# tud-amr/semantic_dsp_map

Measured on AMD Instinct MI355X. Metric: Mvoxels updated/sec (256^3 grid, 2M particles, VKITTI2 camera; whole hot-path frame), higher is better.
Workload: dtype f32

## Files before the change

include/sdm.h:

```cpp
#ifndef SDM_H_
#define SDM_H_

#include <stddef.h>
#include <stdint.h>

#ifdef __cplusplus
extern "C" {
#endif

typedef struct sdm_map sdm_map;

typedef enum {
  SDM_OK = 0,
  SDM_ERR_INVALID_ARGUMENT = 1,
  SDM_ERR_NO_DEVICE = 2,
  SDM_ERR_HIP = 3,
  SDM_ERR_CAPACITY = 4,
  SDM_ERR_NOT_CONVERGED = 5,
  SDM_ERR_COMM = 6
} sdm_status;

typedef struct {
  int32_t x_n, y_n, z_n;
  int32_t p_n;
// ... 309 lines not shown
                          const float *w, const uint16_t *ts, const uint16_t *track,
                          const uint8_t *label, const uint8_t *status, const uint8_t *forget,
                          const uint16_t *owner);
sdm_status sdm_get_ck_kappa(sdm_map *m, float *out);
sdm_status sdm_get_bin_counts(sdm_map *m, uint32_t *out);
sdm_status sdm_get_bins(sdm_map *m, uint32_t *out, int64_t cap, int64_t *n_out);
sdm_status sdm_get_extrinsic(sdm_map *m, float *out16);

sdm_status sdm_time_occupancy_sweep(sdm_map *m, int32_t iters, float *avg_ms);
sdm_status sdm_debug_fill_dense(sdm_map *m);
sdm_status sdm_debug_fill_dense_ex(sdm_map *m, int32_t mode);
sdm_status sdm_debug_hinted_groups(sdm_map *m, int64_t *n_out);
sdm_status sdm_debug_sweep_lists(sdm_map *m, int32_t mode);
sdm_status sdm_debug_sweep_mode(sdm_map *m, int32_t *mode_out);
sdm_status sdm_debug_alias_cap(sdm_map *m, int32_t cap);

sdm_status sdm_test_scan(const uint32_t *in, uint32_t *out, int64_t n);
sdm_status sdm_test_sort_pairs(const uint32_t *keys_in, const uint32_t *vals_in, uint32_t *keys_out,
                               uint32_t *vals_out, int64_t n, int32_t nbits);

const char *sdm_last_error(void);
const char *sdm_version(void);

#ifdef __cplusplus
}
#endif
#endif
```

semantic_dsp_map_amd/binding.py:

```python
import ctypes as C
import os

import numpy as np

_HERE = os.path.dirname(os.path.abspath(__file__))
LIB_PATH = os.environ.get("SDM_LIB_PATH") or os.path.join(_HERE, "csrc", "libsdm_hip.so")

LABELED_POINT = np.dtype([("x", "<f4"), ("y", "<f4"), ("z", "<f4"), ("sigma", "<f4"),
                          ("track_id", "<u2"), ("label_id", "u1"), ("is_valid", "u1")])
OBJECT_MOVE = np.dtype([("track_id", "<i4"), ("T", "<f4", (16,))])
VOXEL_RESULT = np.dtype([("wsum", "<f4"), ("track", "<u2"), ("label", "u1"), ("occ", "i1")])
POINT = np.dtype([("x", "<f4"), ("y", "<f4"), ("z", "<f4"), ("track", "<u2"), ("label", "u1"), ("occ", "i1")])
POINT_XYZRGB = np.dtype([("x", "<f4"), ("y", "<f4"), ("z", "<f4"), ("one", "<f4"), ("b", "u1"), ("g", "u1"), ("r", "u1"), ("a", "u1"),
                         ("pad", "<u4", (3,))])
assert LABELED_POINT.itemsize == 20 and OBJECT_MOVE.itemsize == 68 and VOXEL_RESULT.itemsize == 8 and POINT.itemsize == 16
SEGMENT_HIT = np.dtype([("t", "<f4"), ("voxel", "<u4"), ("cells", "<i4"), ("track", "<u2"), ("label", "u1"), ("occ", "i1")])
BOX_RESULT = np.dtype([("n_occupied", "<i4"), ("n_free", "<i4"), ("n_unknown", "<i4"), ("first_occupied", "<u4"), ("clipped", "<i4")])
assert SEGMENT_HIT.itemsize == 16 and BOX_RESULT.itemsize == 20
QUERY_ON_DEVICE = 0x1
QUERY_UNKNOWN_BLOCKS = 0x2
DISTANCE_RESULT = np.dtype([("distance", "<f4"), ("gradient", "<f4", (3,)), ("nearest", "<f4", (3,)), ("d2", "<u4"), ("track", "<u2"),
                            ("label", "u1"), ("occ", "i1")])
assert DISTANCE_RESULT.itemsize == 36
ESDF_UNKNOWN_IS_OBSTACLE = 0x1
# ... 161 lines not shown
        "sdm_load_state": [vp] + [vp] * 10,
        "sdm_get_ck_kappa": [vp, vp],
        "sdm_get_bin_counts": [vp, vp],
        "sdm_get_bins": [vp, vp, i64, C.POINTER(i64)],
        "sdm_get_extrinsic": [vp, vp],
        "sdm_time_occupancy_sweep": [vp, i32, C.POINTER(C.c_float)],
        "sdm_set_issue_mode": [vp, i32],
        "sdm_bind_host_thread": [i32],
        "sdm_host_numa_node_early": [i32],
        "sdm_debug_fill_dense": [vp],
        "sdm_debug_fill_dense_ex": [vp, i32],
        "sdm_debug_hinted_groups": [vp, C.POINTER(C.c_int64)],
        "sdm_debug_sweep_lists": [vp, i32],
        "sdm_debug_sweep_mode": [vp, C.POINTER(i32)],
        "sdm_debug_alias_cap": [vp, i32],
        "sdm_test_scan": [vp, vp, i64],
        "sdm_test_sort_pairs": [vp, vp, vp, vp, i64, i32],
    }
    for name, argtypes in sig.items():
        fn = getattr(L, name)
        fn.argtypes = argtypes
        fn.restype = C.c_int
    L.sdm_last_error.restype = C.c_char_p
    L.sdm_version.restype = C.c_char_p
    global HOST_NUMA_NODE
    HOST_NUMA_NODE = L.sdm_bind_host_thread(int(os.environ.get("LOCAL_RANK", "0")))
    _lib = L
    return L


def _ptr(a):
    if a is None:
# ... 410 lines not shown
    def dump_state(self):
        n = self.v_count * self.S
        st = {k: np.empty(n, dt) for k, dt in STATE_FIELDS}
        _check(self.L, self.L.sdm_dump_state(self.h, *[_ptr(st[k]) for k, _ in STATE_FIELDS]), "sdm_dump_state")
        return st

    def load_state(self, st):
        arrs = [np.ascontiguousarray(st[k], dtype=dt) for k, dt in STATE_FIELDS]
        _check(self.L, self.L.sdm_load_state(self.h, *[_ptr(a) for a in arrs]), "sdm_load_state")

    def ck_kappa(self):
        out = np.empty(self.W * self.H, np.float32)
        _check(self.L, self.L.sdm_get_ck_kappa(self.h, _ptr(out)), "sdm_get_ck_kappa")
        return out.reshape(self.H, self.W)

    def bin_counts(self):
        out = np.empty(self.W * self.H, np.uint32)
        _check(self.L, self.L.sdm_get_bin_counts(self.h, _ptr(out)), "sdm_get_bin_counts")
        return out.reshape(self.H, self.W)

    def bins(self):
        n = C.c_int64()
        _check(self.L, self.L.sdm_get_bins(self.h, None, 0, C.byref(n)), "sdm_get_bins")
        out = np.empty(max(n.value, 1), np.uint32)
        _check(self.L, self.L.sdm_get_bins(self.h, _ptr(out), n.value, C.byref(n)), "sdm_get_bins")
        return out[:n.value]

    def extrinsic(self):
        out = np.empty(16, np.float32)
        _check(self.L, self.L.sdm_get_extrinsic(self.h, _ptr(out)), "sdm_get_extrinsic")
# ... 37 lines not shown
def test_scan(a):
    L = load_library()
    a = np.ascontiguousarray(a, dtype=np.uint32)
    out = np.empty_like(a)
    _check(L, L.sdm_test_scan(_ptr(a), _ptr(out), a.size), "sdm_test_scan")
    return out


def test_sort_pairs(keys, vals, nbits):
    L = load_library()
    keys = np.ascontiguousarray(keys, dtype=np.uint32)
    vals = np.ascontiguousarray(vals, dtype=np.uint32)
    ko, vo = np.empty_like(keys), np.empty_like(vals)
    _check(L, L.sdm_test_sort_pairs(_ptr(keys), _ptr(vals), _ptr(ko), _ptr(vo), keys.size, nbits), "sdm_test_sort_pairs")
    return ko, vo
```

semantic_dsp_map_amd/csrc/debug.hip:

```cpp
#include "sdm_map.h"

namespace {

__global__ void k_spin(unsigned long long ticks, unsigned long long *out) {
  const unsigned long long t0 = wall_clock64();
  out[0] = t0;
  while (wall_clock64() - t0 < ticks) __builtin_amdgcn_s_sleep(8);
  out[1] = wall_clock64();
}
__global__ void k_stamp(unsigned long long *out) { *out = wall_clock64(); }

}

extern "C" {

sdm_status sdm_debug_overlap(sdm_map *m, int32_t which, double out_us[2]) {
  if (!m || which < 0 || which > 2 || !out_us) return SDM_ERR_INVALID_ARGUMENT;
  HIP_TRY(hipSetDevice(m->device));
  unsigned long long *d = nullptr, h[3] = {0, 0, 0};
  DevTemps tmp;
  HIP_TRY(tmp.alloc(&d, 3));
  if (which == 2) HIP_TRY(lazy_stream(m->device, &m->s_moves));
  hipStream_t side = which == 0 ? m->s_frustum : (which == 1 ? m->s_birth : m->s_moves);
  HIP_TRY(hipStreamSynchronize(m->stream));
// ... 66 lines not shown
  m->st.alias_cap = (uint32_t)cap;
  return SDM_OK;
}
sdm_status sdm_debug_hinted_groups(sdm_map *m, int64_t *n_out) {
  if (!m || !n_out) return SDM_ERR_INVALID_ARGUMENT;
  HIP_TRY(hipSetDevice(m->device));
  std::vector<uint8_t> h(grp_hint_bytes(m->d.v_count));
  HIP_TRY(hipMemcpyAsync(h.data(), m->st.grp_hint, h.size(), hipMemcpyDeviceToHost, m->stream));
  HIP_TRY(hipStreamSynchronize(m->stream));
  int64_t n = 0;
  for (uint8_t b : h) n += b != 0;
  *n_out = n;
  return SDM_OK;
}

#ifdef SDM_AB_TIMERS
extern "C++" {
namespace sdm {
void debug_timers(unsigned long long *out32, int reset);
void debug_timers_moves(unsigned long long *out, int reset);
}
}
sdm_status sdm_debug_timers(sdm_map *m, unsigned long long *out32, int reset) {
  HIP_TRY(hipSetDevice(m->device));
  HIP_TRY(hipDeviceSynchronize());
  sdm::debug_timers(out32, reset);
  sdm::debug_timers_moves(out32 + 6 * 8192 * 4, reset);
  return SDM_OK;
}
#endif
// ... 21 lines not shown
  HIP_TRY(tmp.alloc(&ka, (size_t)n));
  HIP_TRY(tmp.alloc(&va, (size_t)n));
  HIP_TRY(tmp.alloc(&kb, (size_t)n));
  HIP_TRY(tmp.alloc(&vb, (size_t)n));
  HIP_TRY(tmp.alloc(&scr, sort_scratch_elems((size_t)n) + 16));
  HIP_TRY(hipMemset(scr, 0, (sort_scratch_elems((size_t)n) + 16) * 4));
  HIP_TRY(hipMemcpy(ka, keys_in, (size_t)n * 4, hipMemcpyHostToDevice));
  HIP_TRY(hipMemcpy(va, vals_in, (size_t)n * 4, hipMemcpyHostToDevice));
  int which = radix_sort_pairs(ka, va, kb, vb, (size_t)n, nbits, scr, nullptr);
  HIP_TRY(hipDeviceSynchronize());
  HIP_TRY(hipMemcpy(keys_out, which ? kb : ka, (size_t)n * 4, hipMemcpyDeviceToHost));
  HIP_TRY(hipMemcpy(vals_out, which ? vb : va, (size_t)n * 4, hipMemcpyDeviceToHost));
  return SDM_OK;
}

}
```

semantic_dsp_map_amd/csrc/kernels.hip:

```cpp
#include <algorithm>

#include <type_traits>

#include <hip/hip_ext.h>
#include "sdm_internal.h"
#include "sdm_scratch.h"

#pragma clang fp contract(off)

namespace sdm {

namespace {

constexpr int TPB = 256;

#ifdef SDM_AB_TIMERS
}
__device__ unsigned long long g_dbg[6][8192 * 4];
namespace {
#define DBG_T() wall_clock64()
#define DBG_PUTK(k, i, v) do { if (blockIdx.x < 8192) g_dbg[k][blockIdx.x * 4 + (i)] = (unsigned long long)(v); } while (0)
#define DBG_PUT(i, v) DBG_PUTK(0, i, v)
#define DBG_LANE0(k, i) do { if (threadIdx.x == 0 && threadIdx.y == 0) DBG_PUTK(k, i, DBG_T()); } while (0)
#else
// ... 1701 lines not shown
                                         const sdm_labeled_point &o, float ck) {
  if (finish) {
    const float ckk = ck * flt.p_detect + flt.noise_number;
    sc.ck_kappa[p] = ckk;
    sc.pix4[p] = make_float4(o.x, o.y, o.z, ckk);
    sc.pixt[p] = (uint32_t)o.track_id | (1u << 16);
  } else {
    ck_out[p] = ck;
  }
}

constexpr int BR_TPB = 640;
constexpr int BR_WAVES = BR_TPB / 64;
constexpr int BR_MAXW = 1 << ROW_COL_BITS;
template <int PPT>
__global__ __launch_bounds__(BR_TPB) __attribute__((amdgpu_waves_per_eu(PPT <= 4 ? 5 : 4, PPT <= 4 ? 5 : 4))) void k_bin_rows(Dims d, State st, Scratch sc) {
  static_assert(PPT == 2 || PPT == 4 || PPT * BR_TPB >= BR_MAXW, "eight pixels per thread cover the widest image");
  __shared__ uint32_t pre[BR_MAXW + 1];
  __shared__ uint32_t wave_tot[BR_WAVES];
  __shared__ uint32_t s_base;
  const int r = blockIdx.x;
  DBG_LANE0(2, 0);
  if (r == (int)gridDim.x - 1 && threadIdx.x < 64) alias_compact_wave(st);
  const bool overflow = sc.cnt->overflow != 0;
  const int lane = threadIdx.x & 63, wid = threadIdx.x >> 6;
  const int W = d.W;
  uint32_t c[PPT];
  const int j0 = PPT * (int)threadIdx.x;
#pragma unroll
  for (int u = 0; u < PPT; ++u) c[u] = (!overflow && j0 + u < W) ? sc.bin_count[r * W + j0 + u] : 0u;
  uint32_t sub_n = 0;
  if (threadIdx.x < ROW_SUBS && !overflow) {
    sub_n = sc.row_cnt[(size_t)(r * ROW_SUBS + threadIdx.x) * ROW_CNT_STRIDE];
    if (sub_n > sc.row_cap) sub_n = sc.row_cap;
  }
  uint32_t inc = 0;
#pragma unroll
  for (int u = 0; u < PPT; ++u) inc += c[u];
  const uint32_t mine = inc;
#pragma unroll
  for (int off = 1; off < 64; off <<= 1) {
    const uint32_t t = __shfl_up(inc, off, 64);
    if (lane >= off) inc += t;
  }
  if (lane == 63) wave_tot[wid] = inc;
  __syncthreads();
  uint32_t before = 0, total = 0;
#pragma unroll
  for (int w = 0; w < BR_WAVES; ++w) {
    if (w < wid) before += wave_tot[w];
    total += wave_tot[w];
  }
  {
    uint32_t run = before + inc - mine;
#pragma unroll
    for (int u = 0; u < PPT; ++u) {
      if (j0 + u < W) pre[j0 + u] = run;
      run += c[u];
    }
  }
  if (threadIdx.x == 0) {
    pre[W] = total;
    s_base = total ? atomicAdd(&sc.cnt->n_vis, total) : 0u;
    if (total && (s_base > sc.cap_vis || total > sc.cap_vis - s_base)) {
      sc.cnt->overflow = 1;
      pre[W] = 0;
    }
  }
  uint32_t sub_ex[ROW_SUBS + 1];
  {
    uint32_t run = 0;
#pragma unroll
    for (int k = 0; k < ROW_SUBS; ++k) {
      sub_ex[k] = run;
      run += (uint32_t)__shfl(sub_n, k, 64);
    }
    sub_ex[ROW_SUBS] = run;
  }
  __shared__ uint32_t s_sub[ROW_SUBS + 1];
  if (threadIdx.x == 0) {
#pragma unroll
    for (int k = 0; k <= ROW_SUBS; ++k) s_sub[k] = sub_ex[k];
  }
  __syncthreads();
  const uint32_t base = s_base;
  uint32_t *__restrict__ bs = sc.bin_start + (size_t)r * (W + 1);
  const bool row_over = total != 0 && pre[W] == 0;
  {
    const int h = d.window_half;
#pragma unroll
    for (int u = 0; u < PPT; ++u) {
      const int j = j0 + u;
      if (j < W) {
        const uint32_t n = row_over ? 0u : pre[j + h + 1 > W ? W : j + h + 1] - pre[j - h < 0 ? 0 : j - h];
        sc.row_win[r * W + j] = (uint8_t)(n > 255u ? 255u : n);
      }
    }
  }
  for (int j = threadIdx.x; j <= W; j += BR_TPB) bs[j] = row_over ? 0u : base + pre[j];
  if (total == 0 || row_over) {
    DBG_LANE0(2, 1);
    return;
  }
  const uint32_t n_row = s_sub[ROW_SUBS];
  for (uint32_t g = threadIdx.x; g < n_row; g += BR_TPB) {
    int sub = 0;
#pragma unroll
    for (int k = 1; k < ROW_SUBS; ++k) sub += s_sub[k] <= g ? 1 : 0;
    const uint2 e = sc.row_list[(size_t)(r * ROW_SUBS + sub) * sc.row_cap + (g - s_sub[sub])];
    sc.bin_idx[base + pre[e.y & (uint32_t)(BR_MAXW - 1)] + (e.y >> ROW_COL_BITS)] = e.x;
  }
  __syncthreads();
  const size_t slot_base = (size_t)d.v_begin << d.p_n;
// ... 70 lines not shown
          a[0] = t;
          sift_down(a, 0, end - 1);
        }
      }
    }
    for (uint32_t i = 0; i < n; ++i) {
      const size_t li = (size_t)a[i] - slot_base;
      const float4 q = st.pos4[li];
      const SlotRef sr = slot_ref_li(st, d.p_n, li);
      sc.vp4[s + i] = make_float4(q.x, q.y, q.z, sr.w());
      sc.vtf[s + i] = (uint32_t)sr.track() | ((uint32_t)st.forget[li] << 16);
      sc.vpix[s + i] = p;
    }
  }
  DBG_LANE0(2, 1);
}

__global__ __launch_bounds__(TPB) void k_ck_classify(Dims d, Filter flt, Scratch sc, float *__restrict__ ck_out, int finish) {
  const uint32_t p = blockIdx.x * blockDim.x + threadIdx.x;
  const int W = d.W, H = d.H, h = d.window_half;
  const bool in_image = p < (uint32_t)(W * H);
  const bool overflow = sc.cnt->overflow != 0;
  sdm_labeled_point o;
  o.is_valid = 0;
  uint32_t total = 0;
  if (in_image) {
    o = load_point(sc.fa->cloud, p);
    const int i = (int)p / W;
    uint32_t rw[A7_ROWS];
#pragma unroll
    for (int r = 0; r < A7_ROWS; ++r) {
      const int ni = i + r - h;
      const bool ok = r <= 2 * h && ni >= 0 && ni < H;
      rw[r] = sc.row_win[(int)p + (ok ? (r - h) * W : 0)];
    }
    __builtin_amdgcn_sched_barrier(0);
#pragma unroll
    for (int r = 0; r < A7_ROWS; ++r) {
      const int ni = i + r - h;
      total += (r <= 2 * h && ni >= 0 && ni < H) ? rw[r] : 0u;
    }
  }
  uint8_t cls = CK_DONE;
  if (in_image && o.is_valid && total != 0 && !overflow) cls = total <= CK_LIGHT_MAX ? CK_LIGHT : CK_HEAVY;
  const unsigned long long hm = __ballot(cls == CK_HEAVY);
  if (hm) {
    const uint32_t lane = threadIdx.x & 63u;
    const uint32_t shard = blockIdx.x & (VIS_SHARDS - 1);
    uint32_t base = 0;
    if (lane == 0) base = atomicAdd(&sc.cnt->shard[shard].heavy, (uint32_t)__popcll(hm));
    base = (uint32_t)__shfl((int)base, 0, 64);
    if (cls == CK_HEAVY) sc.ck_heavy[shard * sc.cap_heavy + base + (uint32_t)__popcll(hm & ((1ull << lane) - 1ull))] = p;
  }
  if (!in_image) return;
  if (!finish) {
    sc.pix4[p] = make_float4(o.x, o.y, o.z, 0.f);
    sc.pixt[p] = o.is_valid ? ((uint32_t)o.track_id | (1u << 16)) : 0u;
  }
  if (!o.is_valid) {
    if (finish) sc.pixt[p] = 0;
  } else if (cls == CK_DONE) {
    ck_store(flt, sc, ck_out, finish, (int)p, o, 0.f);
  }
  sc.ck_class[p] = cls;
}


template <bool FAST>
__device__ __forceinline__ float ck_term(const Filter &flt, const float *__restrict__ pdf, const float4 pv, const uint32_t tf,
                                         const sdm_labeled_point &o, float rsig, bool &skip) {
  const uint16_t ptrack = (uint16_t)(tf & 0xffffu);
  skip = flt.independent && ptrack != o.track_id;
  const float fg = flt.forget[(tf >> 16) & 7];
  float gk = query_pdf_r<FAST>(pdf, pv.x, o.x, o.sigma, rsig) * query_pdf_r<FAST>(pdf, pv.y, o.y, o.sigma, rsig) *
             query_pdf_r<FAST>(pdf, pv.z, o.z, o.sigma, rsig);
  if (!flt.independent) {
    gk *= fg;
    if (ptrack != o.track_id) gk *= flt.id_transition;
  }
// ... 411 lines not shown
  if (pt.is_valid) {
    if (flt.use_rng) {
      long long draw = (long long)sc.cur->birth_cursor + 3ll * ((long long)flt.nb * sc.b_rank[q] + n);
      float nx = pt.sigma * st.noise[(draw + 1) % flt.noise_n];
      float ny = pt.sigma * st.noise[(draw + 2) % flt.noise_n];
      float nz = pt.sigma * st.noise[(draw + 3) % flt.noise_n];
      x = pt.x + nx;
      y = pt.y + ny;
      z = pt.z + nz;
    }
    uint32_t rx, ry, rz;
    uint32_t v = global_pos_to_voxel(d, f, x, y, z, rx, ry, rz);
    if (v != INVALID_INDEX && rz >= d.rz_begin && rz < d.rz_begin + d.rz_count) key = v;
  }
  sc.bkey_a[b] = key;
  sc.bval_a[b] = b;
  sc.bpos[b] = make_float4(x, y, z, __uint_as_float((uint32_t)pt.track_id | ((uint32_t)pt.label_id << 16)));
}

__global__ void k_birth_cursor(Dims d, Filter flt, Scratch sc) {
  if (threadIdx.x != 0 || blockIdx.x != 0) return;
  int last = d.W * d.H - 1;
  uint32_t n_valid = sc.b_rank[last] + sc.b_valid[last];
  sc.cnt->n_valid_px = n_valid;
  sc.cnt->n_birth_attempts = n_valid * (uint32_t)flt.nb;
  if (flt.use_rng) {
    long long c = (long long)sc.cur->birth_cursor + 3ll * flt.nb * (long long)n_valid;
    sc.cur->birth_cursor = (int32_t)(c % flt.noise_n);
  }
}

// ... 863 lines not shown
                       hipEvent_t vis_done) {
  {
    const size_t max_words = (size_t)((d.NX + 63) / 64 + 1) * d.NY * d.NZ;
    dim3 grid((unsigned)std::min<size_t>(blocks_for(max_words, VIS_WORDS), 2048));
    if (vis_done) {
      switch (d.p_n) {
        case 1: hipExtLaunchKernelGGL(k_visibility<2>, grid, dim3(TPB), 0, s, nullptr, vis_done, 0, d, st, sc); break;
        case 2: hipExtLaunchKernelGGL(k_visibility<4>, grid, dim3(TPB), 0, s, nullptr, vis_done, 0, d, st, sc); break;
        case 3: hipExtLaunchKernelGGL(k_visibility<8>, grid, dim3(TPB), 0, s, nullptr, vis_done, 0, d, st, sc); break;
        default: hipExtLaunchKernelGGL(k_visibility<16>, grid, dim3(TPB), 0, s, nullptr, vis_done, 0, d, st, sc); break;
      }
    } else {
      SDM_DISPATCH_S(k_visibility, grid, s, d, st, sc);
    }
  }
  if (d.W <= 2 * BR_TPB) hipLaunchKernelGGL(k_bin_rows<2>, dim3((unsigned)d.H), dim3(BR_TPB), 0, s, d, st, sc);
  else if (d.W <= 4 * BR_TPB) hipLaunchKernelGGL(k_bin_rows<4>, dim3((unsigned)d.H), dim3(BR_TPB), 0, s, d, st, sc);
  else hipLaunchKernelGGL(k_bin_rows<8>, dim3((unsigned)d.H), dim3(BR_TPB), 0, s, d, st, sc);
  hipLaunchKernelGGL(k_ck_classify, dim3(blocks_for((size_t)d.W * d.H)), dim3(TPB), 0, s, d, flt, sc, ck_out, finish);
}

void launch_ck(const Dims &d, const Filter &flt, const State &st, const Scratch &sc, float *ck_out, int finish, hipStream_t s) {
  hipLaunchKernelGGL(k_ck, dim3(CK_HEAVY_BLOCKS + blocks_for((size_t)d.W * d.H, A7_ROWS * A7_ITEMS)), dim3(A7_ROWS, A7_ITEMS), 0, s, d, flt, st, sc,
                     ck_out, finish);
}
void launch_ck_finish(const Dims &d, const Filter &flt, const Scratch &sc, const float *parts, int n_parts, size_t part_stride, hipStream_t s) {
  hipLaunchKernelGGL(k_ck_finish, dim3(blocks_for((size_t)d.W * d.H)), dim3(TPB), 0, s, d, flt, sc, parts, n_parts,
                     part_stride ? part_stride : (size_t)d.W * d.H);
}
void launch_ck_reduce_chunk(const float *stage, const float *own_part, float *full, uint32_t chunk, int world, int rank, hipStream_t s) {
  hipLaunchKernelGGL(k_ck_reduce_chunk, dim3((chunk + TPB - 1) / TPB), dim3(TPB), 0, s, stage, own_part, full, chunk, world, rank);
}
void launch_weight(const Dims &d, const Filter &flt, const State &st, const Scratch &sc, hipStream_t s, const float *ck_raw) {
  const int side = 2 * d.window_half + 1;
// ... 9 lines not shown
  }
#undef SDM_WEIGHT
}

int launch_birth_prepare(const Dims &d, const Filter &flt, const BirthOrder &bo, const State &st,
                         const Scratch &sc, hipStream_t s) {
  const size_t hw = (size_t)d.W * d.H;
  const size_t total = hw * flt.nb;
  if (flt.use_rng) {
    hipLaunchKernelGGL(k_birth_flags, dim3(blocks_for(hw)), dim3(TPB), 0, s, d, bo, sc);
    exclusive_scan_u32(sc.b_valid, sc.b_rank, hw, sc.scan_scratch_b, s);
  }
  hipLaunchKernelGGL(k_birth_candidates, dim3(blocks_for(total)), dim3(TPB), 0, s, d, flt, bo, st, sc);
  if (flt.use_rng) hipLaunchKernelGGL(k_birth_cursor, dim3(1), dim3(64), 0, s, d, flt, sc);
  int nbits = d.x_n + d.y_n + d.z_n + 1;
  return radix_sort_pairs(sc.bkey_a, sc.bval_a, sc.bkey_b, sc.bval_b, total, nbits, sc.sort_scratch, s);
}

void launch_birth_replay(const Dims &d, const Filter &flt, const State &st, const Scratch &sc, int which, bool literal,
                         hipStream_t s) {
  const size_t total = (size_t)d.W * d.H * flt.nb;
  const uint32_t *skey = which ? sc.bkey_b : sc.bkey_a;
  const uint32_t *sval = which ? sc.bval_b : sc.bval_a;
  dim3 grid(blocks_for(total));
#define SDM_BIRTH(SS)                                                                                                  \
  if (literal) hipLaunchKernelGGL((k_birth_replay<SS, true>), grid, dim3(TPB), 0, s, d, flt, st, sc, skey, sval, (uint32_t)total); \
  else hipLaunchKernelGGL((k_birth_replay<SS, false>), grid, dim3(TPB), 0, s, d, flt, st, sc, skey, sval, (uint32_t)total);
  switch (d.p_n) {
    case 1: SDM_BIRTH(2) break;
    case 2: SDM_BIRTH(4) break;
    case 3: SDM_BIRTH(8) break;
// ... 167 lines not shown
```

semantic_dsp_map_amd/csrc/lifecycle.hip:

```cpp
#include <rocrand/rocrand.h>

#include <chrono>
#include <cmath>
#include <cstdlib>
#include <mutex>

#include "sdm_map.h"

#pragma clang fp contract(off)

namespace {

thread_local std::string g_last_error;

__attribute__((constructor(101))) void sdm_runtime_defaults() {
  setenv("HIP_FORCE_DEV_KERNARG", "1", 0);
}

constexpr double GRAPH_PIECES_US = 110.0, GRAPH_CHAIN_US = 170.0;
constexpr int LAUNCHES_PER_FRAME = 50;

__global__ void k_noop() {}

}
// ... 428 lines not shown
  }
  Scratch &sc = m->sc;
  sc.wpl = (int)((d.NX + 1 + 63) / 64);
  const size_t n_words = (size_t)(d.NZ + 1) * (d.NY + 1) * sc.wpl;
  A(sc.vmask, n_words);
  A(sc.reach, n_words);
  sc.wy = (int)((d.NY + 1 + 63) / 64);
  const size_t n_line_words = (size_t)(d.NZ + 1) * sc.wy;
  A(sc.line_ne, n_line_words);
  A(sc.line_ey, n_line_words);
  A(sc.line_ez, n_line_words);
  A(sc.line_reach, n_line_words);
  A(m->d_depth, hw);
  A(m->d_cloud, hw);
  A(sc.bin_count, hw + 1 + (size_t)d.H * ROW_SUBS * ROW_CNT_STRIDE);
  A(sc.row_win, hw);
  sc.row_cnt = sc.bin_count + hw + 1;
  A(sc.bin_start, (size_t)d.H * (d.W + 1));
  size_t cap_vis = cfg->max_visible > 0 ? (size_t)cfg->max_visible
                                        : std::min<size_t>(n_slots + (size_t)VIS_SHARDS * 256 * d.S, (size_t)16 << 20);
  cap_vis = (cap_vis + VIS_SHARDS - 1) / VIS_SHARDS * VIS_SHARDS;
  cap_vis = std::min<size_t>(cap_vis, 0xffffff00u);
  sc.cap_vis = (uint32_t)cap_vis;
  {
    const size_t row_total = std::min<size_t>(cap_vis, std::max<size_t>(2 * cap_vis / (size_t)d.H, (size_t)2 * d.W * d.S));
    sc.row_cap = (uint32_t)std::max<size_t>(64, (row_total + row_total / 4) / ROW_SUBS + 64);
  }
  A(sc.row_list, (size_t)d.H * ROW_SUBS * sc.row_cap);
  A(sc.bin_idx, cap_vis);
  A(sc.vpix, cap_vis);
  A(sc.vp4, cap_vis);
  A(sc.vtf, cap_vis);
  A(sc.pix4, hw);
  A(sc.pixt, hw);
  A(sc.ck_kappa, hw);
  sc.cap_heavy = (uint32_t)(((hw + 255) / 256 + VIS_SHARDS - 1) / VIS_SHARDS * 256);
  A(sc.ck_heavy, (size_t)sc.cap_heavy * VIS_SHARDS);
  A(sc.ck_class, hw);
  m->ck_chunk = (uint32_t)(((hw + shard_count - 1) / shard_count + 63) / 64 * 64);
  A(m->d_ck_part, (size_t)m->ck_chunk * shard_count);
  for (auto &r : m->raw) {
    A(r.depth, hw);
    A(r.static_mask, hw);
    A(r.label_to_inst, 256);
    A(r.bbox, 6 * MAX_CLOUD_OBJECTS);
  }
  A(sc.b_valid, hw + 1);
  A(sc.b_rank, hw + 1);
  sc.cap_move = (uint32_t)std::min<size_t>((size_t)d.V * d.S, (size_t)1 << 18);
  A(m->d_counts_local, HALO_OBJ);
  const size_t mv_cnt_n = move_count_elems();
// ... 221 lines not shown
```

semantic_dsp_map_amd/csrc/primitives.hip:

```cpp
#include "sdm_internal.h"

namespace sdm {

namespace {

constexpr int SCAN_THREADS = 256;
constexpr int SCAN_ITEMS = 8;
constexpr int SCAN_TILE = SCAN_THREADS * SCAN_ITEMS;

__device__ __forceinline__ uint32_t wave_inclusive_scan(uint32_t v) {
  const int lane = threadIdx.x & 63;
#pragma unroll
  for (int off = 1; off < 64; off <<= 1) {
    uint32_t n = __shfl_up(v, off, 64);
    if (lane >= off) v += n;
  }
  return v;
}

__device__ __forceinline__ uint32_t block_exclusive_scan(uint32_t v, uint32_t *total) {
  __shared__ uint32_t wave_sums[SCAN_THREADS / 64];
  const int lane = threadIdx.x & 63, wid = threadIdx.x >> 6;
  uint32_t inc = wave_inclusive_scan(v);
  if (lane == 63) wave_sums[wid] = inc;
// ... 128 lines not shown
  __syncthreads();
  size_t base = (size_t)blockIdx.x * RS_TILE;
#pragma unroll
  for (int r = 0; r < RS_ITEMS; ++r) {
    size_t k = base + (size_t)r * RS_THREADS + threadIdx.x;
    if (k < n) atomicAdd(&h[(keys[k] >> shift) & (RS_RADIX - 1)], 1u);
  }
  __syncthreads();
#pragma unroll
  for (int q = 0; q < RS_DPT; ++q) {
    int dg = threadIdx.x + q * RS_THREADS;
    hist[(size_t)dg * n_tiles + blockIdx.x] = h[dg];
  }
}

__global__ __launch_bounds__(RS_THREADS) void rs_scatter(const uint32_t *__restrict__ keys_in,
                                                         const uint32_t *__restrict__ vals_in,
                                                         uint32_t *__restrict__ keys_out, uint32_t *__restrict__ vals_out,
                                                         const uint32_t *__restrict__ offsets, size_t n, int shift,
                                                         uint32_t n_tiles, const uint32_t *__restrict__ n_dev) {
  __shared__ uint32_t digit_base[RS_RADIX];
  __shared__ uint32_t wave_cnt[RS_WAVES][RS_RADIX];
  if (n_dev) n = *n_dev < n ? (size_t)*n_dev : n;
  if ((size_t)blockIdx.x * RS_TILE >= n) return;
  const int lane = threadIdx.x & 63, wid = threadIdx.x >> 6;
#pragma unroll
  for (int q = 0; q < RS_DPT; ++q) {
    int dg = threadIdx.x + q * RS_THREADS;
    digit_base[dg] = offsets[(size_t)dg * n_tiles + blockIdx.x];
  }
  size_t base = (size_t)blockIdx.x * RS_TILE;
  const uint64_t lt_mask = (lane == 0) ? 0ull : (~0ull >> (64 - lane));
  for (int r = 0; r < RS_ITEMS; ++r) {
#pragma unroll
    for (int w = 0; w < RS_WAVES; ++w)
#pragma unroll
      for (int q = 0; q < RS_DPT; ++q) wave_cnt[w][threadIdx.x + q * RS_THREADS] = 0;
    __syncthreads();
    size_t k = base + (size_t)r * RS_THREADS + threadIdx.x;
    bool valid = k < n;
    uint32_t key = valid ? keys_in[k] : 0u;
    uint32_t val = valid ? vals_in[k] : 0u;
    uint32_t digit = (key >> shift) & (RS_RADIX - 1);
    uint64_t peers = __ballot(valid);
#pragma unroll
    for (int b = 0; b < RS_BITS; ++b) {
      bool bit = (digit >> b) & 1u;
      uint64_t m = __ballot(bit);
      peers &= bit ? m : ~m;
    }
    uint32_t rank_in_wave = (uint32_t)__popcll(peers & lt_mask);
    if (valid && rank_in_wave == 0) wave_cnt[wid][digit] = (uint32_t)__popcll(peers);
    __syncthreads();
    if (valid) {
      uint32_t off = digit_base[digit] + rank_in_wave;
#pragma unroll
      for (int w = 0; w < RS_WAVES; ++w)
// ... 31 lines not shown
    return;
  }
  hipLaunchKernelGGL(scan_tile_sums, dim3((unsigned)tiles), dim3(SCAN_THREADS), 0, s, in, scratch, n, n_dev);
  hipLaunchKernelGGL(scan_tiles, dim3((unsigned)tiles), dim3(SCAN_THREADS), 0, s, in, out, scratch, n, n_dev);
}

constexpr size_t RS_SCAN_REGION = 2 * (size_t)SCAN_ONEPASS_MAX_TILES + 8;
size_t sort_scratch_elems(size_t n) {
  size_t tiles = (n + RS_TILE - 1) / RS_TILE;
  size_t hist = (size_t)RS_RADIX * tiles;
  size_t scan_tiles = (hist + SCAN_TILE - 1) / SCAN_TILE;
  return RS_SCAN_REGION + hist + (scan_tiles > (size_t)SCAN_ONEPASS_MAX_TILES ? scan_tiles + 1 : 0);
}

int radix_sort_pairs(uint32_t *keys_a, uint32_t *vals_a, uint32_t *keys_b, uint32_t *vals_b, size_t n, int nbits,
                     uint32_t *scratch, hipStream_t s, const uint32_t *n_dev) {
  if (n == 0) return 0;
  size_t tiles = (n + RS_TILE - 1) / RS_TILE;
  size_t hist_n = (size_t)RS_RADIX * tiles;
  uint32_t *hist = scratch + RS_SCAN_REGION;
  const size_t scan_tiles = (hist_n + SCAN_TILE - 1) / SCAN_TILE;
  uint32_t *scan_scratch = scan_tiles > (size_t)SCAN_ONEPASS_MAX_TILES ? hist + hist_n : scratch;
  int which = 0;
  for (int shift = 0; shift < nbits; shift += RS_BITS) {
    uint32_t *kin = which ? keys_b : keys_a, *vin = which ? vals_b : vals_a;
    uint32_t *kout = which ? keys_a : keys_b, *vout = which ? vals_a : vals_b;
    hipLaunchKernelGGL(rs_histogram, dim3((unsigned)tiles), dim3(RS_THREADS), 0, s, kin, hist, n, shift, (uint32_t)tiles, n_dev);
    exclusive_scan_u32(hist, hist, hist_n, scan_scratch, s, nullptr);
    hipLaunchKernelGGL(rs_scatter, dim3((unsigned)tiles), dim3(RS_THREADS), 0, s, kin, vin, kout, vout, hist, n, shift,
                       (uint32_t)tiles, n_dev);
    which ^= 1;
  }
  return which;
}

}
```

semantic_dsp_map_amd/csrc/sdm_internal.h:

```cpp
#pragma once
#include <hip/hip_runtime.h>
#include <stdint.h>

#include "../../include/sdm.h"

#pragma clang fp contract(off)

namespace sdm {

constexpr uint32_t INVALID_INDEX = 0xffffffffu;
constexpr uint16_t OWNER_NONE = 0xFFFF;
constexpr int PDF_NUM = 20000;
#define SDM_OCC_INIT_WEIGHT 0.05f
#define SDM_MIN_RIGHT_PDF 0.1f

enum : uint8_t { ST_INVALID = 0, ST_UPDATED = 1, ST_REGULAR_BORN = 2, ST_GUESSED_BORN = 3, ST_COPIED = 4, ST_TIMEPTC = 5 };

struct Dims {
  int x_n, y_n, z_n, p_n;
  uint32_t NX, NY, NZ, S;
  uint32_t V;
  uint32_t v_begin;
  uint32_t v_count;
  uint32_t rz_begin, rz_count;
// ... 442 lines not shown
  if ((fl & VR_MASK) != VR_UNOBSERVED) {
    sdm_voxel_result out;
    out.wsum = -1.f;
    out.track = 0;
    out.label = 0;
    out.occ = -1;
    store_result(st.res + lv, out);
  }
}


size_t scan_scratch_elems(size_t n);
void exclusive_scan_u32(const uint32_t *in, uint32_t *out, size_t n, uint32_t *scratch, hipStream_t s, const uint32_t *n_dev = nullptr);
size_t sort_scratch_elems(size_t n);
int radix_sort_pairs(uint32_t *keys_a, uint32_t *vals_a, uint32_t *keys_b, uint32_t *vals_b, size_t n, int nbits,
                     uint32_t *scratch, hipStream_t s, const uint32_t *n_dev = nullptr);

void launch_clear(const Dims &d, const State &st, hipStream_t s, bool fresh);

void launch_query_points(const Dims &d, const Frame &f, const State &st, const float *xyz, uint32_t n, sdm_voxel_result *out,
                         uint32_t *voxel_out, hipStream_t s);
void launch_query_segments(const Dims &d, const Frame &f, const State &st, const float *ab, uint32_t n, sdm_segment_hit *out,
                           int unknown_blocks, hipStream_t s);
void launch_query_boxes(const Dims &d, const Frame &f, const State &st, const float *boxes, uint32_t n, sdm_box_result *out,
                        hipStream_t s);

hipError_t launch_esdf_build(const Dims &d, const Frame &f, const State &st, uint32_t flags, uint32_t *site, uint32_t *snap,
                             hipStream_t s);
void launch_query_distance(const Dims &d, const Frame &f, const uint32_t *site, const uint32_t *snap, const float *xyz, uint32_t n,
                           sdm_distance_result *out, hipStream_t s);

// ... 2 lines not shown
```

semantic_dsp_map_amd/csrc/sdm_scratch.h:

```cpp
#pragma once
#include "sdm_internal.h"

namespace sdm {

struct BirthOrder {
  int off[10];
  int cols[9];
};

struct MoveCopy {
  float x, y, z;
  uint32_t forget_bits;
  float w;
  uint16_t ts, track, owner;
  uint8_t label, status;
  uint32_t voxel;
};
static_assert(sizeof(MoveCopy) == 32, "MoveCopy layout");

constexpr int MAX_MOVE_OBJECTS = 48;
constexpr int MAX_REMOVE_TRACKS = 128;
constexpr int HALO_OBJ = 64;
constexpr int HALO_RECORD_BYTES = 36;
constexpr int HALO_HEADER_BYTES = 16;
// ... 20 lines not shown
static_assert(sizeof(FrameArgs) <= 3400, "FrameArgs travels as a kernel argument (4 KB limit, with the launch's other arguments)");

constexpr int MV_ROW = 16;
constexpr int MV_DIRECT = MV_ROW - 2;
constexpr uint32_t MV_FIRST = 0x100u;
struct Scratch {
  const FrameArgs *fa = nullptr;
  const FrameArgs *fa_side = nullptr;
  const FrameArgs *fa_moves = nullptr;
  uint64_t *vmask = nullptr, *reach = nullptr;
  int wpl = 0;
  uint64_t *line_ne = nullptr, *line_ey = nullptr, *line_ez = nullptr, *line_reach = nullptr;
  int wy = 0;
  uint32_t *bin_count = nullptr, *bin_start = nullptr;
  uint32_t *row_cnt = nullptr;
  uint8_t *row_win = nullptr;
  uint2 *row_list = nullptr;
  uint32_t row_cap = 0;
  uint32_t cap_vis = 0;
  uint32_t *bin_idx = nullptr, *vpix = nullptr;
  float4 *vp4 = nullptr;
  uint32_t *vtf = nullptr;
  float4 *pix4 = nullptr;
  uint32_t *pixt = nullptr;
  float *ck_kappa = nullptr;
  uint8_t *ck_class = nullptr;
  uint32_t *ck_heavy = nullptr;
  uint32_t cap_heavy = 0;
  uint32_t *b_valid = nullptr, *b_rank = nullptr;
  uint32_t *bkey_a = nullptr, *bval_a = nullptr, *bkey_b = nullptr, *bval_b = nullptr;
  float4 *bpos = nullptr;
// ... 120 lines not shown
```

Baseline: 95640.

## Fuse CK classification into row binning and synthesize iota sort values

Merges the separate k_ck_classify kernel into k_bin_rows. Each row block now reads the vertical window of bin counts directly, builds a windowed prefix sum in shared memory, classifies its pixels, writes pix4/pixt and the heavy-pixel lists, and drops the row_win byte plane along with one launch. Separately, the birth radix sort no longer writes iota values in k_birth_candidates; the first scatter pass generates them from the element index. The trade-off is extra loads and registers in k_bin_rows (A7_ROWS reads per pixel) and a resized heavy-list capacity. Debug and test entry points are also added.

Result: no change. 95580 (-0.1%).

```diff
diff --git a/include/sdm.h b/include/sdm.h
--- a/include/sdm.h
+++ b/include/sdm.h
@@ -347,10 +347,14 @@
 sdm_status sdm_debug_sweep_lists(sdm_map *m, int32_t mode);
 sdm_status sdm_debug_sweep_mode(sdm_map *m, int32_t *mode_out);
 sdm_status sdm_debug_alias_cap(sdm_map *m, int32_t cap);
+sdm_status sdm_debug_ck_classes(sdm_map *m, uint8_t *cls, uint32_t *heavy, int64_t heavy_cap, int64_t *n_heavy,
+                                float *pix4, uint32_t *pixt);
 
 sdm_status sdm_test_scan(const uint32_t *in, uint32_t *out, int64_t n);
 sdm_status sdm_test_sort_pairs(const uint32_t *keys_in, const uint32_t *vals_in, uint32_t *keys_out,
                                uint32_t *vals_out, int64_t n, int32_t nbits);
+sdm_status sdm_test_sort_sequence(const uint32_t *keys_in, uint32_t *keys_out, uint32_t *vals_out, const int64_t *n,
+                                  int32_t count, int32_t nbits);
 
 const char *sdm_last_error(void);
 const char *sdm_version(void);
diff --git a/semantic_dsp_map_amd/binding.py b/semantic_dsp_map_amd/binding.py
--- a/semantic_dsp_map_amd/binding.py
+++ b/semantic_dsp_map_amd/binding.py
@@ -199,8 +199,10 @@
         "sdm_debug_sweep_lists": [vp, i32],
         "sdm_debug_sweep_mode": [vp, C.POINTER(i32)],
         "sdm_debug_alias_cap": [vp, i32],
+        "sdm_debug_ck_classes": [vp, vp, vp, i64, C.POINTER(i64), vp, vp],
         "sdm_test_scan": [vp, vp, i64],
         "sdm_test_sort_pairs": [vp, vp, vp, vp, i64, i32],
+        "sdm_test_sort_sequence": [vp, vp, vp, vp, i32, i32],
     }
     for name, argtypes in sig.items():
         fn = getattr(L, name)
@@ -641,6 +643,16 @@
         _check(self.L, self.L.sdm_get_ck_kappa(self.h, _ptr(out)), "sdm_get_ck_kappa")
         return out.reshape(self.H, self.W)
 
+    def ck_classes(self, operands=False):
+        hw = self.W * self.H
+        cls, heavy, n = np.empty(hw, np.uint8), np.empty(hw, np.uint32), C.c_int64()
+        pix4 = np.empty((hw, 4), np.float32) if operands else None
+        pixt = np.empty(hw, np.uint32) if operands else None
+        _check(self.L, self.L.sdm_debug_ck_classes(self.h, _ptr(cls), _ptr(heavy), hw, C.byref(n), _ptr(pix4), _ptr(pixt)),
+               "sdm_debug_ck_classes")
+        assert n.value <= hw, n.value
+        return (cls, heavy[:n.value], pix4, pixt) if operands else (cls, heavy[:n.value])
+
     def bin_counts(self):
         out = np.empty(self.W * self.H, np.uint32)
         _check(self.L, self.L.sdm_get_bin_counts(self.h, _ptr(out)), "sdm_get_bin_counts")
@@ -708,3 +720,13 @@
     ko, vo = np.empty_like(keys), np.empty_like(vals)
     _check(L, L.sdm_test_sort_pairs(_ptr(keys), _ptr(vals), _ptr(ko), _ptr(vo), keys.size, nbits), "sdm_test_sort_pairs")
     return ko, vo
+
+
+def test_sort_sequence(key_arrays, nbits):
+    L = load_library()
+    sizes = np.array([len(k) for k in key_arrays], np.int64)
+    keys = np.ascontiguousarray(np.concatenate(key_arrays), dtype=np.uint32)
+    ko, vo = np.empty_like(keys), np.empty_like(keys)
+    _check(L, L.sdm_test_sort_sequence(_ptr(keys), _ptr(ko), _ptr(vo), _ptr(sizes), sizes.size, nbits), "sdm_test_sort_sequence")
+    ends = np.cumsum(sizes)
+    return [(ko[e - n:e], vo[e - n:e]) for n, e in zip(sizes, ends)]
diff --git a/semantic_dsp_map_amd/csrc/debug.hip b/semantic_dsp_map_amd/csrc/debug.hip
--- a/semantic_dsp_map_amd/csrc/debug.hip
+++ b/semantic_dsp_map_amd/csrc/debug.hip
@@ -104,6 +104,31 @@
   return SDM_OK;
 }
 
+sdm_status sdm_debug_ck_classes(sdm_map *m, uint8_t *cls, uint32_t *heavy, int64_t heavy_cap, int64_t *n_heavy, float *pix4, uint32_t *pixt) {
+  if (!m || !cls || !n_heavy || heavy_cap < 0 || (heavy_cap > 0 && !heavy)) return SDM_ERR_INVALID_ARGUMENT;
+  HIP_TRY(hipSetDevice(m->device));
+  const size_t hw = (size_t)m->d.W * m->d.H;
+  Counters c;
+  std::vector<uint32_t> lists((size_t)m->sc.cap_heavy * VIS_SHARDS);
+  HIP_TRY(hipMemcpyAsync(&c, m->sc.cnt, sizeof(c), hipMemcpyDeviceToHost, m->stream));
+  HIP_TRY(hipMemcpyAsync(cls, m->sc.ck_class, hw, hipMemcpyDeviceToHost, m->stream));
+  HIP_TRY(hipMemcpyAsync(lists.data(), m->sc.ck_heavy, lists.size() * 4, hipMemcpyDeviceToHost, m->stream));
+  if (pix4) HIP_TRY(hipMemcpyAsync(pix4, m->sc.pix4, hw * 16, hipMemcpyDeviceToHost, m->stream));
+  if (pixt) HIP_TRY(hipMemcpyAsync(pixt, m->sc.pixt, hw * 4, hipMemcpyDeviceToHost, m->stream));
+  HIP_TRY(hipStreamSynchronize(m->stream));
+  int64_t n = 0;
+  for (uint32_t sh = 0; sh < VIS_SHARDS; ++sh) {
+    if (c.shard[sh].heavy > m->sc.cap_heavy) {
+      set_error("sdm_debug_ck_classes", __FILE__, __LINE__, "a heavy-pixel list is longer than its capacity");
+      return SDM_ERR_CAPACITY;
+    }
+    for (uint32_t k = 0; k < c.shard[sh].heavy; ++k, ++n)
+      if (n < heavy_cap) heavy[n] = lists[(size_t)sh * m->sc.cap_heavy + k];
+  }
+  *n_heavy = n;
+  return SDM_OK;
+}
+
 #ifdef SDM_AB_TIMERS
 extern "C++" {
 namespace sdm {
@@ -155,4 +180,33 @@
   return SDM_OK;
 }
 
-}
+sdm_status sdm_test_sort_sequence(const uint32_t *keys_in, uint32_t *keys_out, uint32_t *vals_out, const int64_t *n, int32_t count,
+                                  int32_t nbits) {
+  if (!keys_in || !keys_out || !vals_out || !n || count <= 0 || nbits <= 0 || nbits > 32) return SDM_ERR_INVALID_ARGUMENT;
+  int64_t n_max = 0;
+  for (int i = 0; i < count; ++i) {
+    if (n[i] <= 0) return SDM_ERR_INVALID_ARGUMENT;
+    n_max = std::max(n_max, n[i]);
+  }
+  uint32_t *ka, *va, *kb, *vb, *scr;
+  DevTemps tmp;
+  HIP_TRY(tmp.alloc(&ka, (size_t)n_max));
+  HIP_TRY(tmp.alloc(&va, (size_t)n_max));
+  HIP_TRY(tmp.alloc(&kb, (size_t)n_max));
+  HIP_TRY(tmp.alloc(&vb, (size_t)n_max));
+  HIP_TRY(tmp.alloc(&scr, sort_scratch_elems((size_t)n_max) + 16));
+  HIP_TRY(hipMemset(scr, 0, (sort_scratch_elems((size_t)n_max) + 16) * 4));
+  int64_t at = 0;
+  for (int i = 0; i < count; ++i) {
+    HIP_TRY(hipMemcpy(ka, keys_in + at, (size_t)n[i] * 4, hipMemcpyHostToDevice));
+    HIP_TRY(hipMemset(va, 0xff, (size_t)n_max * 4));
+    int which = radix_sort_pairs(ka, va, kb, vb, (size_t)n[i], nbits, scr, nullptr, nullptr, true);
+    HIP_TRY(hipDeviceSynchronize());
+    HIP_TRY(hipMemcpy(keys_out + at, which ? kb : ka, (size_t)n[i] * 4, hipMemcpyDeviceToHost));
+    HIP_TRY(hipMemcpy(vals_out + at, which ? vb : va, (size_t)n[i] * 4, hipMemcpyDeviceToHost));
+    at += n[i];
+  }
+  return SDM_OK;
+}
+
+}
diff --git a/semantic_dsp_map_amd/csrc/kernels.hip b/semantic_dsp_map_amd/csrc/kernels.hip
--- a/semantic_dsp_map_amd/csrc/kernels.hip
+++ b/semantic_dsp_map_amd/csrc/kernels.hip
@@ -1739,17 +1739,19 @@
 constexpr int BR_WAVES = BR_TPB / 64;
 constexpr int BR_MAXW = 1 << ROW_COL_BITS;
 template <int PPT>
-__global__ __launch_bounds__(BR_TPB) __attribute__((amdgpu_waves_per_eu(PPT <= 4 ? 5 : 4, PPT <= 4 ? 5 : 4))) void k_bin_rows(Dims d, State st, Scratch sc) {
+__global__ __launch_bounds__(BR_TPB) __attribute__((amdgpu_waves_per_eu(PPT <= 4 ? 5 : 4, PPT <= 4 ? 5 : 4))) void k_bin_rows(Dims d, Filter flt, State st, Scratch sc,
+                                                                                                                       float *__restrict__ ck_out, int finish) {
   static_assert(PPT == 2 || PPT == 4 || PPT * BR_TPB >= BR_MAXW, "eight pixels per thread cover the widest image");
   __shared__ uint32_t pre[BR_MAXW + 1];
-  __shared__ uint32_t wave_tot[BR_WAVES];
+  __shared__ uint32_t win[BR_MAXW + 1];
+  __shared__ uint32_t wave_tot[BR_WAVES], wave_win[BR_WAVES];
   __shared__ uint32_t s_base;
   const int r = blockIdx.x;
   DBG_LANE0(2, 0);
   if (r == (int)gridDim.x - 1 && threadIdx.x < 64) alias_compact_wave(st);
   const bool overflow = sc.cnt->overflow != 0;
   const int lane = threadIdx.x & 63, wid = threadIdx.x >> 6;
-  const int W = d.W;
+  const int W = d.W, H = d.H, h = d.window_half;
   uint32_t c[PPT];
   const int j0 = PPT * (int)threadIdx.x;
 #pragma unroll
@@ -1759,33 +1761,77 @@
     sub_n = sc.row_cnt[(size_t)(r * ROW_SUBS + threadIdx.x) * ROW_CNT_STRIDE];
     if (sub_n > sc.row_cap) sub_n = sc.row_cap;
   }
-  uint32_t inc = 0;
-#pragma unroll
-  for (int u = 0; u < PPT; ++u) inc += c[u];
-  const uint32_t mine = inc;
+  uint32_t cs[PPT];
+#pragma unroll
+  for (int u0 = 0; u0 < PPT; u0 += 2) {
+    uint32_t rw[2][A7_ROWS];
+#pragma unroll
+    for (int u = 0; u < 2; ++u) {
+      const int j = j0 + u0 + u < W ? j0 + u0 + u : 0;
+#pragma unroll
+      for (int k = 0; k < A7_ROWS; ++k) {
+        const int ni = r + k - h;
+        const bool ok = k <= 2 * h && ni >= 0 && ni < H;
+        rw[u][k] = sc.bin_count[(ok ? ni : r) * W + j];
+      }
+    }
+    __builtin_amdgcn_sched_barrier(0);
+#pragma unroll
+    for (int u = 0; u < 2; ++u) {
+      uint32_t sum = 0;
+#pragma unroll
+      for (int k = 0; k < A7_ROWS; ++k) {
+        const int ni = r + k - h;
+        sum += (k <= 2 * h && ni >= 0 && ni < H) ? rw[u][k] : 0u;
+      }
+      cs[u0 + u] = (!overflow && j0 + u0 + u < W) ? sum : 0u;
+    }
+  }
+  uint32_t inc = 0, winc = 0;
+#pragma unroll
+  for (int u = 0; u < PPT; ++u) {
+    inc += c[u];
+    winc += cs[u];
+  }
+  const uint32_t mine = inc, wmine = winc;
 #pragma unroll
   for (int off = 1; off < 64; off <<= 1) {
-    const uint32_t t = __shfl_up(inc, off, 64);
-    if (lane >= off) inc += t;
-  }
-  if (lane == 63) wave_tot[wid] = inc;
+    const uint32_t t = __shfl_up(inc, off, 64), tw = __shfl_up(winc, off, 64);
+    if (lane >= off) {
+      inc += t;
+      winc += tw;
+    }
+  }
+  if (lane == 63) {
+    wave_tot[wid] = inc;
+    wave_win[wid] = winc;
+  }
   __syncthreads();
-  uint32_t before = 0, total = 0;
+  uint32_t before = 0, total = 0, wbefore = 0, wtotal = 0;
 #pragma unroll
   for (int w = 0; w < BR_WAVES; ++w) {
-    if (w < wid) before += wave_tot[w];
+    if (w < wid) {
+      before += wave_tot[w];
+      wbefore += wave_win[w];
+    }
     total += wave_tot[w];
+    wtotal += wave_win[w];
   }
   {
-    uint32_t run = before + inc - mine;
+    uint32_t run = before + inc - mine, wrun = wbefore + winc - wmine;
 #pragma unroll
     for (int u = 0; u < PPT; ++u) {
-      if (j0 + u < W) pre[j0 + u] = run;
+      if (j0 + u < W) {
+        pre[j0 + u] = run;
+        win[j0 + u] = wrun;
+      }
       run += c[u];
+      wrun += cs[u];
     }
   }
   if (threadIdx.x == 0) {
     pre[W] = total;
+    win[W] = wtotal;
     s_base = total ? atomicAdd(&sc.cnt->n_vis, total) : 0u;
     if (total && (s_base > sc.cap_vis || total > sc.cap_vis - s_base)) {
       sc.cnt->overflow = 1;
@@ -1807,21 +1853,59 @@
 #pragma unroll
     for (int k = 0; k <= ROW_SUBS; ++k) s_sub[k] = sub_ex[k];
   }
+  sdm_labeled_point o[PPT];
+#pragma unroll
+  for (int u = 0; u < PPT; ++u) {
+    o[u].is_valid = 0;
+    if (j0 + u < W) o[u] = load_point(sc.fa->cloud, (size_t)(r * W + j0 + u));
+  }
   __syncthreads();
   const uint32_t base = s_base;
+  {
+    uint8_t cls[PPT];
+    unsigned long long hm[PPT];
+    uint32_t n_heavy = 0;
+#pragma unroll
+    for (int u = 0; u < PPT; ++u) {
+      const int j = j0 + u;
+      cls[u] = CK_DONE;
+      if (j < W) {
+        const uint32_t n = win[j + h + 1 > W ? W : j + h + 1] - win[j - h < 0 ? 0 : j - h];
+        if (o[u].is_valid && n != 0) cls[u] = n <= CK_LIGHT_MAX ? CK_LIGHT : CK_HEAVY;
+      }
+      hm[u] = __ballot(cls[u] == CK_HEAVY);
+      n_heavy += (uint32_t)__popcll(hm[u]);
+    }
+    const uint32_t shard = (uint32_t)r & (VIS_SHARDS - 1);
+    uint32_t place = 0;
+    if (n_heavy) {
+      if (lane == 0) place = atomicAdd(&sc.cnt->shard[shard].heavy, n_heavy);
+      place = (uint32_t)__shfl((int)place, 0, 64);
+    }
+#pragma unroll
+    for (int u = 0; u < PPT; ++u) {
+      const int j = j0 + u;
+      if (j >= W) continue;
+      const int p = r * W + j;
+      if (!finish) {
+        sc.pix4[p] = make_float4(o[u].x, o[u].y, o[u].z, 0.f);
+        sc.pixt[p] = o[u].is_valid ? ((uint32_t)o[u].track_id | (1u << 16)) : 0u;
+      }
+      if (!o[u].is_valid) {
+        if (finish) sc.pixt[p] = 0;
+      } else if (cls[u] == CK_DONE) {
+        ck_store(flt, sc, ck_out, finish, p, o[u], 0.f);
+      }
+      sc.ck_class[p] = cls[u];
+    }
+#pragma unroll
+    for (int u = 0; u < PPT; ++u) {
+      if (cls[u] == CK_HEAVY) sc.ck_heavy[shard * sc.cap_heavy + place + (uint32_t)__popcll(hm[u] & ((1ull << lane) - 1ull))] = (uint32_t)(r * W + j0 + u);
+      place += (uint32_t)__popcll(hm[u]);
+    }
+  }
   uint32_t *__restrict__ bs = sc.bin_start + (size_t)r * (W + 1);
   const bool row_over = total != 0 && pre[W] == 0;
-  {
-    const int h = d.window_half;
-#pragma unroll
-    for (int u = 0; u < PPT; ++u) {
-      const int j = j0 + u;
-      if (j < W) {
-        const uint32_t n = row_over ? 0u : pre[j + h + 1 > W ? W : j + h + 1] - pre[j - h < 0 ? 0 : j - h];
-        sc.row_win[r * W + j] = (uint8_t)(n > 255u ? 255u : n);
-      }
-    }
-  }
   for (int j = threadIdx.x; j <= W; j += BR_TPB) bs[j] = row_over ? 0u : base + pre[j];
   if (total == 0 || row_over) {
     DBG_LANE0(2, 1);
@@ -1922,55 +2006,6 @@
     }
   }
   DBG_LANE0(2, 1);
-}
-
-__global__ __launch_bounds__(TPB) void k_ck_classify(Dims d, Filter flt, Scratch sc, float *__restrict__ ck_out, int finish) {
-  const uint32_t p = blockIdx.x * blockDim.x + threadIdx.x;
-  const int W = d.W, H = d.H, h = d.window_half;
-  const bool in_image = p < (uint32_t)(W * H);
-  const bool overflow = sc.cnt->overflow != 0;
-  sdm_labeled_point o;
-  o.is_valid = 0;
-  uint32_t total = 0;
-  if (in_image) {
-    o = load_point(sc.fa->cloud, p);
-    const int i = (int)p / W;
-    uint32_t rw[A7_ROWS];
-#pragma unroll
-    for (int r = 0; r < A7_ROWS; ++r) {
-      const int ni = i + r - h;
-      const bool ok = r <= 2 * h && ni >= 0 && ni < H;
-      rw[r] = sc.row_win[(int)p + (ok ? (r - h) * W : 0)];
-    }
-    __builtin_amdgcn_sched_barrier(0);
-#pragma unroll
-    for (int r = 0; r < A7_ROWS; ++r) {
-      const int ni = i + r - h;
-      total += (r <= 2 * h && ni >= 0 && ni < H) ? rw[r] : 0u;
-    }
-  }
-  uint8_t cls = CK_DONE;
-  if (in_image && o.is_valid && total != 0 && !overflow) cls = total <= CK_LIGHT_MAX ? CK_LIGHT : CK_HEAVY;
-  const unsigned long long hm = __ballot(cls == CK_HEAVY);
-  if (hm) {
-    const uint32_t lane = threadIdx.x & 63u;
-    const uint32_t shard = blockIdx.x & (VIS_SHARDS - 1);
-    uint32_t base = 0;
-    if (lane == 0) base = atomicAdd(&sc.cnt->shard[shard].heavy, (uint32_t)__popcll(hm));
-    base = (uint32_t)__shfl((int)base, 0, 64);
-    if (cls == CK_HEAVY) sc.ck_heavy[shard * sc.cap_heavy + base + (uint32_t)__popcll(hm & ((1ull << lane) - 1ull))] = p;
-  }
-  if (!in_image) return;
-  if (!finish) {
-    sc.pix4[p] = make_float4(o.x, o.y, o.z, 0.f);
-    sc.pixt[p] = o.is_valid ? ((uint32_t)o.track_id | (1u << 16)) : 0u;
-  }
-  if (!o.is_valid) {
-    if (finish) sc.pixt[p] = 0;
-  } else if (cls == CK_DONE) {
-    ck_store(flt, sc, ck_out, finish, (int)p, o, 0.f);
-  }
-  sc.ck_class[p] = cls;
 }
 
 
@@ -2412,7 +2447,6 @@
     if (v != INVALID_INDEX && rz >= d.rz_begin && rz < d.rz_begin + d.rz_count) key = v;
   }
   sc.bkey_a[b] = key;
-  sc.bval_a[b] = b;
   sc.bpos[b] = make_float4(x, y, z, __uint_as_float((uint32_t)pt.track_id | ((uint32_t)pt.label_id << 16)));
 }
 
@@ -3306,10 +3340,9 @@
       SDM_DISPATCH_S(k_visibility, grid, s, d, st, sc);
     }
   }
-  if (d.W <= 2 * BR_TPB) hipLaunchKernelGGL(k_bin_rows<2>, dim3((unsigned)d.H), dim3(BR_TPB), 0, s, d, st, sc);
-  else if (d.W <= 4 * BR_TPB) hipLaunchKernelGGL(k_bin_rows<4>, dim3((unsigned)d.H), dim3(BR_TPB), 0, s, d, st, sc);
-  else hipLaunchKernelGGL(k_bin_rows<8>, dim3((unsigned)d.H), dim3(BR_TPB), 0, s, d, st, sc);
-  hipLaunchKernelGGL(k_ck_classify, dim3(blocks_for((size_t)d.W * d.H)), dim3(TPB), 0, s, d, flt, sc, ck_out, finish);
+  if (d.W <= 2 * BR_TPB) hipLaunchKernelGGL(k_bin_rows<2>, dim3((unsigned)d.H), dim3(BR_TPB), 0, s, d, flt, st, sc, ck_out, finish);
+  else if (d.W <= 4 * BR_TPB) hipLaunchKernelGGL(k_bin_rows<4>, dim3((unsigned)d.H), dim3(BR_TPB), 0, s, d, flt, st, sc, ck_out, finish);
+  else hipLaunchKernelGGL(k_bin_rows<8>, dim3((unsigned)d.H), dim3(BR_TPB), 0, s, d, flt, st, sc, ck_out, finish);
 }
 
 void launch_ck(const Dims &d, const Filter &flt, const State &st, const Scratch &sc, float *ck_out, int finish, hipStream_t s) {
@@ -3349,7 +3382,7 @@
   hipLaunchKernelGGL(k_birth_candidates, dim3(blocks_for(total)), dim3(TPB), 0, s, d, flt, bo, st, sc);
   if (flt.use_rng) hipLaunchKernelGGL(k_birth_cursor, dim3(1), dim3(64), 0, s, d, flt, sc);
   int nbits = d.x_n + d.y_n + d.z_n + 1;
-  return radix_sort_pairs(sc.bkey_a, sc.bval_a, sc.bkey_b, sc.bval_b, total, nbits, sc.sort_scratch, s);
+  return radix_sort_pairs(sc.bkey_a, sc.bval_a, sc.bkey_b, sc.bval_b, total, nbits, sc.sort_scratch, s, nullptr, true);
 }
 
 void launch_birth_replay(const Dims &d, const Filter &flt, const State &st, const Scratch &sc, int which, bool literal,
diff --git a/semantic_dsp_map_amd/csrc/lifecycle.hip b/semantic_dsp_map_amd/csrc/lifecycle.hip
--- a/semantic_dsp_map_amd/csrc/lifecycle.hip
+++ b/semantic_dsp_map_amd/csrc/lifecycle.hip
@@ -466,7 +466,6 @@
   A(m->d_depth, hw);
   A(m->d_cloud, hw);
   A(sc.bin_count, hw + 1 + (size_t)d.H * ROW_SUBS * ROW_CNT_STRIDE);
-  A(sc.row_win, hw);
   sc.row_cnt = sc.bin_count + hw + 1;
   A(sc.bin_start, (size_t)d.H * (d.W + 1));
   size_t cap_vis = cfg->max_visible > 0 ? (size_t)cfg->max_visible
@@ -486,7 +485,7 @@
   A(sc.pix4, hw);
   A(sc.pixt, hw);
   A(sc.ck_kappa, hw);
-  sc.cap_heavy = (uint32_t)(((hw + 255) / 256 + VIS_SHARDS - 1) / VIS_SHARDS * 256);
+  sc.cap_heavy = (uint32_t)(((size_t)d.H + VIS_SHARDS - 1) / VIS_SHARDS * (size_t)d.W);
   A(sc.ck_heavy, (size_t)sc.cap_heavy * VIS_SHARDS);
   A(sc.ck_class, hw);
   m->ck_chunk = (uint32_t)(((hw + shard_count - 1) / shard_count + 63) / 64 * 64);
diff --git a/semantic_dsp_map_amd/csrc/primitives.hip b/semantic_dsp_map_amd/csrc/primitives.hip
--- a/semantic_dsp_map_amd/csrc/primitives.hip
+++ b/semantic_dsp_map_amd/csrc/primitives.hip
@@ -166,6 +166,7 @@
   }
 }
 
+template <bool IOTA>
 __global__ __launch_bounds__(RS_THREADS) void rs_scatter(const uint32_t *__restrict__ keys_in,
                                                          const uint32_t *__restrict__ vals_in,
                                                          uint32_t *__restrict__ keys_out, uint32_t *__restrict__ vals_out,
@@ -192,7 +193,9 @@
     size_t k = base + (size_t)r * RS_THREADS + threadIdx.x;
     bool valid = k < n;
     uint32_t key = valid ? keys_in[k] : 0u;
-    uint32_t val = valid ? vals_in[k] : 0u;
+    uint32_t val;
+    if constexpr (IOTA) val = (uint32_t)k;
+    else val = valid ? vals_in[k] : 0u;
     uint32_t digit = (key >> shift) & (RS_RADIX - 1);
     uint64_t peers = __ballot(valid);
 #pragma unroll
@@ -254,7 +257,7 @@
 }
 
 int radix_sort_pairs(uint32_t *keys_a, uint32_t *vals_a, uint32_t *keys_b, uint32_t *vals_b, size_t n, int nbits,
-                     uint32_t *scratch, hipStream_t s, const uint32_t *n_dev) {
+                     uint32_t *scratch, hipStream_t s, const uint32_t *n_dev, bool vals_iota) {
   if (n == 0) return 0;
   size_t tiles = (n + RS_TILE - 1) / RS_TILE;
   size_t hist_n = (size_t)RS_RADIX * tiles;
@@ -267,8 +270,10 @@
     uint32_t *kout = which ? keys_a : keys_b, *vout = which ? vals_a : vals_b;
     hipLaunchKernelGGL(rs_histogram, dim3((unsigned)tiles), dim3(RS_THREADS), 0, s, kin, hist, n, shift, (uint32_t)tiles, n_dev);
     exclusive_scan_u32(hist, hist, hist_n, scan_scratch, s, nullptr);
-    hipLaunchKernelGGL(rs_scatter, dim3((unsigned)tiles), dim3(RS_THREADS), 0, s, kin, vin, kout, vout, hist, n, shift,
-                       (uint32_t)tiles, n_dev);
+    if (shift == 0 && vals_iota)
+      hipLaunchKernelGGL(rs_scatter<true>, dim3((unsigned)tiles), dim3(RS_THREADS), 0, s, kin, vin, kout, vout, hist, n, shift, (uint32_t)tiles, n_dev);
+    else
+      hipLaunchKernelGGL(rs_scatter<false>, dim3((unsigned)tiles), dim3(RS_THREADS), 0, s, kin, vin, kout, vout, hist, n, shift, (uint32_t)tiles, n_dev);
     which ^= 1;
   }
   return which;
diff --git a/semantic_dsp_map_amd/csrc/sdm_internal.h b/semantic_dsp_map_amd/csrc/sdm_internal.h
--- a/semantic_dsp_map_amd/csrc/sdm_internal.h
+++ b/semantic_dsp_map_amd/csrc/sdm_internal.h
@@ -480,7 +480,7 @@
 void exclusive_scan_u32(const uint32_t *in, uint32_t *out, size_t n, uint32_t *scratch, hipStream_t s, const uint32_t *n_dev = nullptr);
 size_t sort_scratch_elems(size_t n);
 int radix_sort_pairs(uint32_t *keys_a, uint32_t *vals_a, uint32_t *keys_b, uint32_t *vals_b, size_t n, int nbits,
-                     uint32_t *scratch, hipStream_t s, const uint32_t *n_dev = nullptr);
+                     uint32_t *scratch, hipStream_t s, const uint32_t *n_dev = nullptr, bool vals_iota = false);
 
 void launch_clear(const Dims &d, const State &st, hipStream_t s, bool fresh);
 
diff --git a/semantic_dsp_map_amd/csrc/sdm_scratch.h b/semantic_dsp_map_amd/csrc/sdm_scratch.h
--- a/semantic_dsp_map_amd/csrc/sdm_scratch.h
+++ b/semantic_dsp_map_amd/csrc/sdm_scratch.h
@@ -58,7 +58,6 @@
   int wy = 0;
   uint32_t *bin_count = nullptr, *bin_start = nullptr;
   uint32_t *row_cnt = nullptr;
-  uint8_t *row_win = nullptr;
   uint2 *row_list = nullptr;
   uint32_t row_cap = 0;
   uint32_t cap_vis = 0;
```
